# praveer13/zest

Measured on AMD Instinct MI355X. Metric: aggregate pull GB/s + P2P ratio, Llama-3.1-70B at 1/2/4/8 MI355X peers, higher is better.
Workload: dtype bf16

## Files before the change

csrc/gpu/compress.hip:

```cpp
#include <hip/hip_runtime.h>

#include <cstdint>
#include <cstdlib>

#include "zgpu.h"

namespace {

constexpr int kWave = 64;
constexpr int kWavesPerBlock = 4;
constexpr int kTabLog = 12;
constexpr uint32_t kTab = 1u << kTabLog;

__device__ __forceinline__ uint32_t lane_id() { return threadIdx.x & (kWave - 1); }

__device__ __forceinline__ uint32_t load_u32(const uint8_t* p) {
  const uintptr_t a = reinterpret_cast<uintptr_t>(p);
  const uint32_t k = uint32_t(a & 3);
  const uint32_t* w = reinterpret_cast<const uint32_t*>(a & ~uintptr_t(3));
  const uint32_t w0 = w[0];
  return k == 0 ? w0 : __builtin_amdgcn_alignbyte(w[1], w0, k);
}

__device__ __forceinline__ uint32_t put_len(uint8_t* o, uint32_t op, uint32_t r, uint32_t lane) {
  const uint32_t nff = r / 255;
  for (uint32_t i = lane; i < nff; i += kWave) o[op + i] = 0xFF;
  if (lane == 0) o[op + nff] = uint8_t(r - 255 * nff);
  return op + nff + 1;
}

__device__ __forceinline__ uint32_t emit(uint8_t* o, uint32_t op, const uint8_t* in, uint32_t lit0, uint32_t L,
                                         uint32_t off, uint32_t ml, uint32_t lane) {
  const uint32_t M = ml ? ml - 4 : 0;
  if (lane == 0) o[op] = uint8_t(((L < 15 ? L : 15) << 4) | (ml ? (M < 15 ? M : 15) : 0));
  ++op;
  if (L >= 15) op = put_len(o, op, L - 15, lane);
  for (uint32_t i = lane; i < L; i += kWave) o[op + i] = in[lit0 + i];
  op += L;
  if (ml) {
    if (lane == 0) {
      o[op] = uint8_t(off & 0xFF);
      o[op + 1] = uint8_t(off >> 8);
    }
    op += 2;
    if (M >= 15) op = put_len(o, op, M - 15, lane);
  }
  return op;
}

__global__ void __launch_bounds__(256) k_bg4_split(const uint8_t* __restrict__ data, const uint64_t* __restrict__ offs,
                                                   const uint32_t* __restrict__ lens, int n, uint8_t* __restrict__ out,
                                                   uint64_t slot) {
  const int c = __builtin_amdgcn_readfirstlane(int(blockIdx.x * kWavesPerBlock + (threadIdx.x >> 6)));
  if (c >= n) return;
  const uint32_t lane = lane_id(), len = lens[c];
  const uint8_t* s = data + offs[c];
  uint8_t* d = out + uint64_t(c) * slot;
  const uint32_t q = len >> 2, r = len & 3;
  const uint32_t g1 = q + (r > 0), g2 = g1 + q + (r > 1), g3 = g2 + q + (r > 2);
  for (uint32_t i = lane; i < len; i += kWave) {
    const uint32_t g = i & 3, j = i >> 2;
    const uint32_t base = g == 0 ? 0u : g == 1 ? g1 : g == 2 ? g2 : g3;
    d[base + j] = s[i];
  }
}

__global__ void __launch_bounds__(256) k_lz4_compress_v1(const uint8_t* __restrict__ data, const uint64_t* __restrict__ offs,
                                                      const uint32_t* __restrict__ lens, int n, uint64_t in_slot,
                                                      uint8_t* __restrict__ out, uint64_t out_slot,
                                                      uint32_t* __restrict__ out_len, uint32_t hc64, uint32_t hc256) {
  __shared__ unsigned long long tabs[kWavesPerBlock][kTab];
  const int wave = __builtin_amdgcn_readfirstlane(int(threadIdx.x >> 6));
  const int c = __builtin_amdgcn_readfirstlane(int(blockIdx.x * kWavesPerBlock + wave));
  if (c >= n) return;
  const uint32_t lane = lane_id();
  unsigned long long* tab = tabs[wave];
  for (uint32_t i = lane; i < kTab; i += kWave) tab[i] = 0;
  __builtin_amdgcn_wave_barrier();
  const uint32_t len = lens[c];
  const uint8_t* in = in_slot ? data + uint64_t(c) * in_slot : data + offs[c];
  uint8_t* o = out + uint64_t(c) * out_slot;
  uint32_t op = 11, ip = 0, anchor = 0;
  const uint32_t mend = len > 5 ? len - 5 : 0;
  while (ip + 12 <= len) {
    const uint32_t p = ip + lane;
    const bool ok = p + 12 <= len;
    const uint32_t v = ok ? load_u32(in + p) : 0;
    const uint32_t h = (v * 2654435761u) >> (32 - kTabLog);
    const unsigned long long e = ok ? tab[h] : 0ull;
    uint32_t cand = uint32_t(e >> 32) - 1;
    bool hit = ok && e != 0 && uint32_t(e) == v && cand < p && p - cand <= 65535u;
    uint32_t near = 0;
    for (int d = 32; d >= 1; --d) {
      const uint32_t u = __shfl_up(v, d, kWave);
      if (lane >= uint32_t(d) && u == v) near = d;
    }
    if (ok && near) {
      cand = p - near;
      hit = true;
    }
    const unsigned long long mask = __ballot(hit);
    const uint32_t passed = mask ? uint32_t(__builtin_ctzll(mask)) + 1 : uint32_t(kWave);
    __builtin_amdgcn_wave_barrier();
    if (ok && lane < passed) atomicMax(&tab[h], (static_cast<unsigned long long>(p + 1) << 32) | v);
    if (!mask) {
      ip += kWave;
      continue;
    }
    const int j = __builtin_ctzll(mask);
    uint32_t mp = ip + uint32_t(j);
    uint32_t mc = uint32_t(__builtin_amdgcn_readlane(int(cand), j));
    while (true) {
      const uint32_t room = (mp - anchor) < mc ? (mp - anchor) : mc;
      if (room == 0) break;
      const uint32_t k = lane + 1;
      const bool eq = k <= room && in[mp - k] == in[mc - k];
      const unsigned long long ne = __ballot(!eq);
      const uint32_t b = ne ? uint32_t(__builtin_ctzll(ne)) : uint32_t(kWave);
      mp -= b;
      mc -= b;
      if (b < uint32_t(kWave)) break;
    }
    const uint32_t maxlen = mend - mp;
    uint32_t ml = 4 + (ip + uint32_t(j) - mp);
    while (ml < maxlen) {
      const uint32_t k = ml + lane;
      const bool eq = k < maxlen && in[mc + k] == in[mp + k];
      const unsigned long long ne = __ballot(!eq);
      if (ne) {
        ml += uint32_t(__builtin_ctzll(ne));
        break;
      }
      ml += kWave;
    }
    if (ml > maxlen) ml = maxlen;
    op = emit(o, op, in, anchor, mp - anchor, mp - mc, ml, lane);
    ip = mp + ml;
    anchor = ip;
  }
  op = emit(o, op, in, anchor, len - anchor, 0, 0, lane);
  const uint32_t total = op + 4;
  if (total >= len) {
    if (lane == 0) out_len[c] = 0;
    return;
  }
  if (lane == 0) {
    const uint32_t bs = op - 11;
    const bool small = len <= 65536;
    const uint8_t hdr[11] = {0x04, 0x22, 0x4D, 0x18, 0x60, uint8_t(small ? 0x40 : 0x50),
                             uint8_t(small ? hc64 : hc256), uint8_t(bs), uint8_t(bs >> 8), uint8_t(bs >> 16),
                             uint8_t(bs >> 24)};
    for (int i = 0; i < 11; ++i) o[i] = hdr[i];
    for (int i = 0; i < 4; ++i) o[op + i] = 0;
    out_len[c] = total;
  }
}

constexpr uint32_t kTagBits = 14;
constexpr uint32_t kTagMask = (1u << kTagBits) - 1;
constexpr uint32_t kRing = 4096;
constexpr uint32_t kRingMask = kRing - 1;
constexpr uint32_t kFlush = 2048;
constexpr uint32_t kHdr = 11;

struct Staged {
  uint8_t* ring;
  uint8_t* g;
  uint32_t flushed;
};

__device__ __forceinline__ void ring_write(Staged& o, uint32_t end, uint32_t lane) {
  __builtin_amdgcn_wave_barrier();
  for (uint32_t pos = o.flushed + lane; pos < end; pos += kWave)
    if (pos >= kHdr) o.g[pos] = o.ring[pos & kRingMask];
  __builtin_amdgcn_wave_barrier();
}

__device__ __forceinline__ void maybe_flush(Staged& o, uint32_t op, uint32_t lane) {
  while (op - o.flushed >= kFlush) {
    ring_write(o, o.flushed + kFlush, lane);
    o.flushed += kFlush;
  }
}

__device__ __forceinline__ uint32_t put_len_s(Staged& o, uint32_t op, uint32_t r, uint32_t lane) {
  const uint32_t nff = r / 255;
  for (uint32_t i = lane; i < nff; i += kWave) o.ring[(op + i) & kRingMask] = 0xFF;
  if (lane == 0) o.ring[(op + nff) & kRingMask] = uint8_t(r - 255 * nff);
  return op + nff + 1;
}

__device__ __forceinline__ uint32_t emit_s(Staged& o, uint32_t op, const uint8_t* in, uint32_t lit0, uint32_t L,
                                           uint32_t off, uint32_t ml, uint32_t lane) {
  const uint32_t M = ml ? ml - 4 : 0;
  maybe_flush(o, op, lane);
  if (lane == 0) o.ring[op & kRingMask] = uint8_t(((L < 15 ? L : 15) << 4) | (ml ? (M < 15 ? M : 15) : 0));
  ++op;
  if (L >= 15) op = put_len_s(o, op, L - 15, lane);
  for (uint32_t b = 0; b < L; b += 1024) {
    maybe_flush(o, op + b, lane);
    const uint32_t n = L - b < 1024 ? L - b : 1024;
    for (uint32_t i = lane; i < n; i += kWave) o.ring[(op + b + i) & kRingMask] = in[lit0 + b + i];
  }
  op += L;
  if (ml) {
    maybe_flush(o, op, lane);
    if (lane == 0) {
      o.ring[op & kRingMask] = uint8_t(off & 0xFF);
      o.ring[(op + 1) & kRingMask] = uint8_t(off >> 8);
    }
    op += 2;
    if (M >= 15) op = put_len_s(o, op, M - 15, lane);
  }
  return op;
}

__global__ void __launch_bounds__(256) k_lz4_compress(const uint8_t* __restrict__ data, const uint64_t* __restrict__ offs,
                                                      const uint32_t* __restrict__ lens, int n, uint64_t in_slot,
                                                      uint8_t* __restrict__ out, uint64_t out_slot,
                                                      uint32_t* __restrict__ out_len, uint32_t hc64, uint32_t hc256) {
  __shared__ uint32_t tabs[kWavesPerBlock][kTab];
  __shared__ uint8_t rings[kWavesPerBlock][kRing];
  const int wave = __builtin_amdgcn_readfirstlane(int(threadIdx.x >> 6));
  const int c = __builtin_amdgcn_readfirstlane(int(blockIdx.x * kWavesPerBlock + wave));
  if (c >= n) return;
  const uint32_t lane = lane_id();
  uint32_t* tab = tabs[wave];
  for (uint32_t i = lane; i < kTab; i += kWave) tab[i] = 0;
  __builtin_amdgcn_wave_barrier();
  const uint32_t len = lens[c];
  const uint8_t* in = in_slot ? data + uint64_t(c) * in_slot : data + offs[c];
  Staged o{rings[wave], out + uint64_t(c) * out_slot, 0};
  uint32_t op = kHdr, ip = 0, anchor = 0;
  const uint32_t mend = len > 5 ? len - 5 : 0;
  while (ip + 12 <= len) {
    const uint32_t p = ip + lane;
    const bool ok = p + 12 <= len;
    const uint32_t v = ok ? load_u32(in + p) : 0;
    const uint32_t hv = v * 2654435761u;
    const uint32_t h = hv >> (32 - kTabLog);
    const uint32_t tag = hv & kTagMask;
    const uint32_t e = ok ? tab[h] : 0u;
    uint32_t cand = (e >> kTagBits) - 1;
    bool hit = ok && e != 0 && (e & kTagMask) == tag && cand < p && p - cand <= 65535u;
    if (hit) hit = load_u32(in + cand) == v;
    uint32_t near = 0;
    for (int d = 32; d >= 1; --d) {
      const uint32_t u = __shfl_up(v, d, kWave);
      if (lane >= uint32_t(d) && u == v) near = d;
    }
    if (ok && near) {
      cand = p - near;
      hit = true;
    }
    const unsigned long long mask = __ballot(hit);
    const uint32_t passed = mask ? uint32_t(__builtin_ctzll(mask)) + 1 : uint32_t(kWave);
    __builtin_amdgcn_wave_barrier();
    if (ok && lane < passed) atomicMax(&tab[h], ((p + 1) << kTagBits) | tag);
    if (!mask) {
      ip += kWave;
      continue;
    }
    const int j = __builtin_ctzll(mask);
    uint32_t mp = ip + uint32_t(j);
    uint32_t mc = uint32_t(__builtin_amdgcn_readlane(int(cand), j));
    while (true) {
      const uint32_t room = (mp - anchor) < mc ? (mp - anchor) : mc;
      if (room == 0) break;
      const uint32_t k = lane + 1;
      const bool eq = k <= room && in[mp - k] == in[mc - k];
      const unsigned long long ne = __ballot(!eq);
      const uint32_t b = ne ? uint32_t(__builtin_ctzll(ne)) : uint32_t(kWave);
      mp -= b;
      mc -= b;
      if (b < uint32_t(kWave)) break;
    }
    const uint32_t maxlen = mend - mp;
    uint32_t ml = 4 + (ip + uint32_t(j) - mp);
    while (ml < maxlen) {
      const uint32_t k = ml + lane;
      const bool eq = k < maxlen && in[mc + k] == in[mp + k];
      const unsigned long long ne = __ballot(!eq);
      if (ne) {
        ml += uint32_t(__builtin_ctzll(ne));
        break;
      }
      ml += kWave;
    }
    if (ml > maxlen) ml = maxlen;
    op = emit_s(o, op, in, anchor, mp - anchor, mp - mc, ml, lane);
    ip = mp + ml;
    anchor = ip;
  }
  op = emit_s(o, op, in, anchor, len - anchor, 0, 0, lane);
  const uint32_t total = op + 4;
  if (total >= len) {
    if (lane == 0) out_len[c] = 0;
    return;
  }
  maybe_flush(o, op, lane);
  if (lane < 4) o.ring[(op + lane) & kRingMask] = 0;
  ring_write(o, total, lane);
  if (lane == 0) {
    const uint32_t bs = op - kHdr;
    const bool small = len <= 65536;
    const uint8_t hdr[kHdr] = {0x04, 0x22, 0x4D, 0x18, 0x60, uint8_t(small ? 0x40 : 0x50),
                               uint8_t(small ? hc64 : hc256), uint8_t(bs), uint8_t(bs >> 8), uint8_t(bs >> 16),
                               uint8_t(bs >> 24)};
    for (uint32_t i = 0; i < kHdr; ++i) o.g[i] = hdr[i];
    out_len[c] = total;
  }
}

bool compress_v1() {
  const char* e = getenv("ZG_COMPRESS");
  return e && e[0] == 'v' && e[1] == '1';
}

__global__ void __launch_bounds__(256) k_pack_frames(const uint64_t* __restrict__ src, const uint32_t* __restrict__ clen,
                                                     const uint32_t* __restrict__ ulen, const uint8_t* __restrict__ scheme,
                                                     const uint64_t* __restrict__ out_off, int n, uint8_t* __restrict__ out) {
  const int c = __builtin_amdgcn_readfirstlane(int(blockIdx.x * kWavesPerBlock + (threadIdx.x >> 6)));
  if (c >= n) return;
  const uint32_t lane = lane_id(), cl = clen[c], ul = ulen[c];
  uint8_t* d = out + out_off[c];
  if (lane < 8) {
    const uint32_t b = lane == 0 ? 0u : lane < 4 ? (cl >> (8 * (lane - 1))) & 0xFF
                                  : lane == 4 ? scheme[c] : (ul >> (8 * (lane - 5))) & 0xFF;
    d[lane] = uint8_t(b);
  }
  const uint8_t* s = reinterpret_cast<const uint8_t*>(src[c]);
  for (uint32_t i = lane; i < cl; i += kWave) d[8 + i] = s[i];
}

}

extern "C" {

hipError_t zg_compress_chunks(const uint8_t* data, const uint64_t* offs, const uint32_t* lens, int n, int bg4,
                              uint8_t* scratch, uint64_t in_slot, uint8_t* out, uint64_t out_slot, uint32_t* out_len,
                              uint32_t hc64, uint32_t hc256, hipStream_t stream) {
  if (n <= 0) return hipSuccess;
  const dim3 grid((n + kWavesPerBlock - 1) / kWavesPerBlock);
  auto* kern = compress_v1() ? k_lz4_compress_v1 : k_lz4_compress;
  if (bg4) {
    hipLaunchKernelGGL(k_bg4_split, grid, dim3(256), 0, stream, data, offs, lens, n, scratch, in_slot);
    hipLaunchKernelGGL(kern, grid, dim3(256), 0, stream, scratch, offs, lens, n, in_slot, out, out_slot, out_len,
                       hc64, hc256);
  } else {
    hipLaunchKernelGGL(kern, grid, dim3(256), 0, stream, data, offs, lens, n, uint64_t(0), out, out_slot, out_len,
                       hc64, hc256);
  }
  return hipGetLastError();
}

hipError_t zg_pack_frames(const uint64_t* src, const uint32_t* clen, const uint32_t* ulen, const uint8_t* scheme,
                          const uint64_t* out_off, int n, uint8_t* out, hipStream_t stream) {
  if (n <= 0) return hipSuccess;
  hipLaunchKernelGGL(k_pack_frames, dim3((n + kWavesPerBlock - 1) / kWavesPerBlock), dim3(256), 0, stream, src, clen,
                     ulen, scheme, out_off, n, out);
  return hipGetLastError();
}

}
```

Baseline: 62.58.

## Stage LZ4 input through LDS ring and batch multiple matches per wave window

The GPU LZ4 compressor now streams each chunk's input through a shared-memory ring, prefetched one refill ahead, so hashing, candidate verification, match extension and literal copies mostly read LDS instead of global memory. The near-match shuffle scan is cut to 8 distances first and only widened when needed. Backward and forward extension use precomputed 4-byte windows before falling back to wave-wide byte loops. Short sequences are emitted in one lane-parallel store, and several matches can be handled per loaded window. Each block now runs one wave instead of four, which changes occupancy and adds more complex control flow with some risk of subtle encoding bugs.

```diff
diff --git a/csrc/gpu/compress.hip b/csrc/gpu/compress.hip
--- a/csrc/gpu/compress.hip
+++ b/csrc/gpu/compress.hip
@@ -190,17 +190,93 @@
   return op + nff + 1;
 }
 
-__device__ __forceinline__ uint32_t emit_s(Staged& o, uint32_t op, const uint8_t* in, uint32_t lit0, uint32_t L,
+#ifndef ZG_LZ4_INRING
+#define ZG_LZ4_INRING 1024
+#endif
+constexpr uint32_t kIn = ZG_LZ4_INRING;
+static_assert(kIn >= 1024 && (kIn & (kIn - 1)) == 0, "input ring: a power of two, at least two refills");
+constexpr uint32_t kInMask = kIn - 1;
+constexpr uint32_t kInDwMask = kIn / 4 - 1;
+constexpr uint32_t kRefill = 512;
+constexpr uint32_t kAhead = 128;
+
+struct Input {
+  const uint8_t* in;
+  const uint32_t* g32;
+  uint32_t* r32;
+  uint32_t k;
+  uint32_t ndw;
+  uint32_t lo, hi;
+  uint32_t pend0, pend1;
+};
+
+__device__ __forceinline__ void in_issue(Input& s, uint32_t lane) {
+  const uint32_t d = (s.hi >> 2) + lane;
+  s.pend0 = d < s.ndw ? s.g32[d] : 0u;
+  s.pend1 = d + kWave < s.ndw ? s.g32[d + kWave] : 0u;
+}
+
+__device__ __forceinline__ void in_commit(Input& s, uint32_t lane) {
+  const uint32_t d = (s.hi >> 2) + lane;
+  s.r32[d & kInDwMask] = s.pend0;
+  s.r32[(d + kWave) & kInDwMask] = s.pend1;
+  s.hi += kRefill;
+  if (s.hi - s.lo > kIn) s.lo = s.hi - kIn;
+  in_issue(s, lane);
+}
+
+__device__ __forceinline__ void in_ensure(Input& s, uint32_t a0, uint32_t lane) {
+  if (a0 > s.hi + kRefill) {
+    s.hi = (a0 - kWave) & ~3u;
+    s.lo = s.hi;
+    in_issue(s, lane);
+  }
+  while (s.hi < a0 + kAhead && s.hi < s.ndw * 4) in_commit(s, lane);
+  __builtin_amdgcn_wave_barrier();
+}
+
+__device__ __forceinline__ uint8_t in_byte(const Input& s, uint32_t p) {
+  const uint32_t a = p + s.k;
+  return (a >= s.lo && a < s.hi) ? reinterpret_cast<const uint8_t*>(s.r32)[a & kInMask] : s.in[p];
+}
+
+struct Cand {
+  uint32_t pre, val, f0, f1;
+};
+
+__device__ __forceinline__ Cand fetch_cand(const Input& s, uint32_t mc, bool want) {
+  const uint32_t a = mc + s.k, d = a >> 2, sh = a & 3;
+  uint32_t c[5];
+#pragma unroll
+  for (uint32_t i = 0; i < 5; ++i) c[i] = s.r32[(d - 1 + i) & kInDwMask];
+  const bool gone = want && (d ? d - 1 : 0u) * 4 < s.lo;
+  if (__ballot(gone)) {
+    if (gone) {
+#pragma unroll
+      for (uint32_t i = 0; i < 5; ++i) c[i] = d - 1 + i < s.ndw ? s.g32[d - 1 + i] : 0u;
+    }
+  }
+  return Cand{__builtin_amdgcn_alignbyte(c[1], c[0], sh), __builtin_amdgcn_alignbyte(c[2], c[1], sh),
+              __builtin_amdgcn_alignbyte(c[3], c[2], sh), __builtin_amdgcn_alignbyte(c[4], c[3], sh)};
+}
+
+__device__ __forceinline__ uint32_t emit_s(Staged& o, uint32_t op, const Input& in, uint32_t lit0, uint32_t L,
                                            uint32_t off, uint32_t ml, uint32_t lane) {
   const uint32_t M = ml ? ml - 4 : 0;
   maybe_flush(o, op, lane);
   if (lane == 0) o.ring[op & kRingMask] = uint8_t(((L < 15 ? L : 15) << 4) | (ml ? (M < 15 ? M : 15) : 0));
   ++op;
   if (L >= 15) op = put_len_s(o, op, L - 15, lane);
+  const uint8_t* r8 = reinterpret_cast<const uint8_t*>(in.r32);
   for (uint32_t b = 0; b < L; b += 1024) {
     maybe_flush(o, op + b, lane);
     const uint32_t n = L - b < 1024 ? L - b : 1024;
-    for (uint32_t i = lane; i < n; i += kWave) o.ring[(op + b + i) & kRingMask] = in[lit0 + b + i];
+    const uint32_t a = lit0 + b + in.k;
+    if (a >= in.lo && a + n <= in.hi) {
+      for (uint32_t i = lane; i < n; i += kWave) o.ring[(op + b + i) & kRingMask] = r8[(a + i) & kInMask];
+    } else {
+      for (uint32_t i = lane; i < n; i += kWave) o.ring[(op + b + i) & kRingMask] = in.in[lit0 + b + i];
+    }
   }
   op += L;
   if (ml) {
@@ -215,84 +291,159 @@
   return op;
 }
 
-__global__ void __launch_bounds__(256) k_lz4_compress(const uint8_t* __restrict__ data, const uint64_t* __restrict__ offs,
-                                                      const uint32_t* __restrict__ lens, int n, uint64_t in_slot,
-                                                      uint8_t* __restrict__ out, uint64_t out_slot,
-                                                      uint32_t* __restrict__ out_len, uint32_t hc64, uint32_t hc256) {
-  __shared__ uint32_t tabs[kWavesPerBlock][kTab];
-  __shared__ uint8_t rings[kWavesPerBlock][kRing];
-  const int wave = __builtin_amdgcn_readfirstlane(int(threadIdx.x >> 6));
-  const int c = __builtin_amdgcn_readfirstlane(int(blockIdx.x * kWavesPerBlock + wave));
+constexpr int kNearFirst = 8;
+
+__global__ void __launch_bounds__(kWave) k_lz4_compress(const uint8_t* __restrict__ data, const uint64_t* __restrict__ offs,
+                                                        const uint32_t* __restrict__ lens, int n, uint64_t in_slot,
+                                                        uint8_t* __restrict__ out, uint64_t out_slot,
+                                                        uint32_t* __restrict__ out_len, uint32_t hc64, uint32_t hc256) {
+  __shared__ uint32_t tab[kTab];
+  __shared__ uint8_t ring[kRing];
+  __shared__ uint32_t inring[kIn / 4];
+  const int c = int(blockIdx.x);
   if (c >= n) return;
-  const uint32_t lane = lane_id();
-  uint32_t* tab = tabs[wave];
+  const uint32_t lane = threadIdx.x;
   for (uint32_t i = lane; i < kTab; i += kWave) tab[i] = 0;
   __builtin_amdgcn_wave_barrier();
   const uint32_t len = lens[c];
   const uint8_t* in = in_slot ? data + uint64_t(c) * in_slot : data + offs[c];
-  Staged o{rings[wave], out + uint64_t(c) * out_slot, 0};
+  Input s;
+  s.in = in;
+  s.k = uint32_t(reinterpret_cast<uintptr_t>(in) & 3);
+  s.g32 = reinterpret_cast<const uint32_t*>(in - s.k);
+  s.r32 = inring;
+  s.ndw = len ? (s.k + len + 3) >> 2 : 0u;
+  s.lo = s.hi = 0;
+  in_issue(s, lane);
+  Staged o{ring, out + uint64_t(c) * out_slot, 0};
   uint32_t op = kHdr, ip = 0, anchor = 0;
   const uint32_t mend = len > 5 ? len - 5 : 0;
   while (ip + 12 <= len) {
-    const uint32_t p = ip + lane;
+    const uint32_t a0 = ip + s.k;
+    in_ensure(s, a0, lane);
+    const uint32_t p = ip + lane, a = a0 + lane, q = a >> 2, sh = a & 3;
     const bool ok = p + 12 <= len;
-    const uint32_t v = ok ? load_u32(in + p) : 0;
+    const uint32_t wm = s.r32[(q - 1) & kInDwMask], w0 = s.r32[q & kInDwMask], w1 = s.r32[(q + 1) & kInDwMask],
+                   w2 = s.r32[(q + 2) & kInDwMask], w3 = s.r32[(q + 3) & kInDwMask];
+    const uint32_t v = __builtin_amdgcn_alignbyte(w1, w0, sh);
     const uint32_t hv = v * 2654435761u;
     const uint32_t h = hv >> (32 - kTabLog);
     const uint32_t tag = hv & kTagMask;
-    const uint32_t e = ok ? tab[h] : 0u;
-    uint32_t cand = (e >> kTagBits) - 1;
-    bool hit = ok && e != 0 && (e & kTagMask) == tag && cand < p && p - cand <= 65535u;
-    if (hit) hit = load_u32(in + cand) == v;
-    uint32_t near = 0;
-    for (int d = 32; d >= 1; --d) {
+    const uint32_t vpre = __builtin_amdgcn_alignbyte(w0, wm, sh), vf0 = __builtin_amdgcn_alignbyte(w2, w1, sh),
+                   vf1 = __builtin_amdgcn_alignbyte(w3, w2, sh);
+    uint32_t near8 = 0;
+#pragma unroll
+    for (int d = kNearFirst; d >= 1; --d) {
       const uint32_t u = __shfl_up(v, d, kWave);
-      if (lane >= uint32_t(d) && u == v) near = d;
-    }
-    if (ok && near) {
-      cand = p - near;
-      hit = true;
-    }
-    const unsigned long long mask = __ballot(hit);
-    const uint32_t passed = mask ? uint32_t(__builtin_ctzll(mask)) + 1 : uint32_t(kWave);
-    __builtin_amdgcn_wave_barrier();
-    if (ok && lane < passed) atomicMax(&tab[h], ((p + 1) << kTagBits) | tag);
-    if (!mask) {
-      ip += kWave;
-      continue;
-    }
-    const int j = __builtin_ctzll(mask);
-    uint32_t mp = ip + uint32_t(j);
-    uint32_t mc = uint32_t(__builtin_amdgcn_readlane(int(cand), j));
+      if (lane >= uint32_t(d) && u == v) near8 = d;
+    }
+    uint32_t s0 = 0;
     while (true) {
+      const bool live = ok && lane >= s0;
+      const uint32_t e = live ? tab[h] : 0u;
+      uint32_t cand = (e >> kTagBits) - 1;
+      const bool tagged = live && e != 0 && (e & kTagMask) == tag && cand < p && p - cand <= 65535u;
+      const Cand cb = fetch_cand(s, cand, tagged);
+      const bool far = tagged && cb.val == v;
+      const unsigned long long mfar = __ballot(far);
+      const uint32_t jf = mfar ? uint32_t(__builtin_ctzll(mfar)) : uint32_t(kWave);
+      uint32_t near = near8 <= lane - s0 ? near8 : 0u;
+      if (jf - s0 > uint32_t(kNearFirst)) {
+        uint32_t nr = 0;
+        for (uint32_t d = jf - s0 < 32 ? jf - s0 : 32; d > uint32_t(kNearFirst); --d) {
+          const uint32_t u = __shfl_up(v, d, kWave);
+          if (lane >= s0 + d && u == v) nr = d;
+        }
+        if (!near) near = nr;
+      }
+      const unsigned long long mask = mfar | __ballot(live && near != 0);
+      if (!mask && s0) {
+        ip += s0;
+        break;
+      }
+      const uint32_t passed = mask ? uint32_t(__builtin_ctzll(mask)) + 1 : uint32_t(kWave);
+      __builtin_amdgcn_wave_barrier();
+      if (live && lane < passed) atomicMax(&tab[h], ((p + 1) << kTagBits) | tag);
+      if (!mask) {
+        ip += kWave;
+        break;
+      }
+      const int j = __builtin_ctzll(mask);
+      uint32_t mp = ip + uint32_t(j);
+      const uint32_t jnear = uint32_t(__builtin_amdgcn_readlane(int(near), j));
+      uint32_t mc;
+      Cand w;
+      if (jnear) {
+        mc = mp - jnear;
+        const Cand t = fetch_cand(s, mc, true);
+        w = Cand{uint32_t(__builtin_amdgcn_readfirstlane(int(t.pre))), 0u, uint32_t(__builtin_amdgcn_readfirstlane(int(t.f0))),
+                 uint32_t(__builtin_amdgcn_readfirstlane(int(t.f1)))};
+      } else {
+        mc = uint32_t(__builtin_amdgcn_readlane(int(cand), j));
+        w = Cand{uint32_t(__builtin_amdgcn_readlane(int(cb.pre), j)), 0u, uint32_t(__builtin_amdgcn_readlane(int(cb.f0), j)),
+                 uint32_t(__builtin_amdgcn_readlane(int(cb.f1), j))};
+      }
       const uint32_t room = (mp - anchor) < mc ? (mp - anchor) : mc;
-      if (room == 0) break;
-      const uint32_t k = lane + 1;
-      const bool eq = k <= room && in[mp - k] == in[mc - k];
-      const unsigned long long ne = __ballot(!eq);
-      const uint32_t b = ne ? uint32_t(__builtin_ctzll(ne)) : uint32_t(kWave);
-      mp -= b;
-      mc -= b;
-      if (b < uint32_t(kWave)) break;
-    }
-    const uint32_t maxlen = mend - mp;
-    uint32_t ml = 4 + (ip + uint32_t(j) - mp);
-    while (ml < maxlen) {
-      const uint32_t k = ml + lane;
-      const bool eq = k < maxlen && in[mc + k] == in[mp + k];
-      const unsigned long long ne = __ballot(!eq);
-      if (ne) {
-        ml += uint32_t(__builtin_ctzll(ne));
+      const uint32_t xb = uint32_t(__builtin_amdgcn_readlane(int(vpre), j)) ^ w.pre;
+      uint32_t nb = xb ? uint32_t(__builtin_clz(xb)) >> 3 : 4u;
+      const bool back_more = nb == 4 && room > 4;
+      if (nb > room) nb = room;
+      mp -= nb;
+      mc -= nb;
+      if (back_more) {
+        while (true) {
+          const uint32_t rm = (mp - anchor) < mc ? (mp - anchor) : mc;
+          if (rm == 0) break;
+          const uint32_t k = lane + 1;
+          const bool eq = k <= rm && in_byte(s, mp - k) == in_byte(s, mc - k);
+          const unsigned long long ne = __ballot(!eq);
+          const uint32_t b = ne ? uint32_t(__builtin_ctzll(ne)) : uint32_t(kWave);
+          mp -= b;
+          mc -= b;
+          if (b < uint32_t(kWave)) break;
+        }
+      }
+      const uint32_t maxlen = mend - mp;
+      uint32_t ml = 4 + (ip + uint32_t(j) - mp);
+      const uint32_t x0 = uint32_t(__builtin_amdgcn_readlane(int(vf0), j)) ^ w.f0;
+      const uint32_t x1 = uint32_t(__builtin_amdgcn_readlane(int(vf1), j)) ^ w.f1;
+      if (x0) {
+        ml += uint32_t(__builtin_ctz(x0)) >> 3;
+      } else if (x1) {
+        ml += 4 + (uint32_t(__builtin_ctz(x1)) >> 3);
+      } else {
+        ml += 8;
+        while (ml < maxlen) {
+          const uint32_t k = ml + lane;
+          const bool eq = k < maxlen && in_byte(s, mc + k) == in_byte(s, mp + k);
+          const unsigned long long ne = __ballot(!eq);
+          if (ne) {
+            ml += uint32_t(__builtin_ctzll(ne));
+            break;
+          }
+          ml += kWave;
+        }
+      }
+      if (ml > maxlen) ml = maxlen;
+      const uint32_t L = mp - anchor, off = mp - mc;
+      if (anchor >= ip && L < 15 && ml < 19) {
+        maybe_flush(o, op, lane);
+        const uint32_t r = (lane - (anchor - ip)) & (kWave - 1);
+        const uint32_t b = r < L ? v : r == L ? ((L << 4) | (ml - 4)) : r == L + 1 ? off : off >> 8;
+        if (r < L + 3) o.ring[(r < L ? op + 1 + r : r == L ? op : op + r) & kRingMask] = uint8_t(b);
+        op += L + 3;
+      } else {
+        op = emit_s(o, op, s, anchor, L, off, ml, lane);
+      }
+      anchor = mp + ml;
+      s0 = anchor - ip;
+      if (s0 > kWave - 20 || anchor + 12 > len) {
+        ip = anchor;
         break;
       }
-      ml += kWave;
-    }
-    if (ml > maxlen) ml = maxlen;
-    op = emit_s(o, op, in, anchor, mp - anchor, mp - mc, ml, lane);
-    ip = mp + ml;
-    anchor = ip;
-  }
-  op = emit_s(o, op, in, anchor, len - anchor, 0, 0, lane);
+    }
+  }
+  op = emit_s(o, op, s, anchor, len - anchor, 0, 0, lane);
   const uint32_t total = op + 4;
   if (total >= len) {
     if (lane == 0) out_len[c] = 0;
@@ -342,15 +493,13 @@
                               uint32_t hc64, uint32_t hc256, hipStream_t stream) {
   if (n <= 0) return hipSuccess;
   const dim3 grid((n + kWavesPerBlock - 1) / kWavesPerBlock);
-  auto* kern = compress_v1() ? k_lz4_compress_v1 : k_lz4_compress;
-  if (bg4) {
-    hipLaunchKernelGGL(k_bg4_split, grid, dim3(256), 0, stream, data, offs, lens, n, scratch, in_slot);
-    hipLaunchKernelGGL(kern, grid, dim3(256), 0, stream, scratch, offs, lens, n, in_slot, out, out_slot, out_len,
-                       hc64, hc256);
-  } else {
-    hipLaunchKernelGGL(kern, grid, dim3(256), 0, stream, data, offs, lens, n, uint64_t(0), out, out_slot, out_len,
-                       hc64, hc256);
-  }
+  const bool v1 = compress_v1();
+  auto* kern = v1 ? k_lz4_compress_v1 : k_lz4_compress;
+  const dim3 kgrid = v1 ? grid : dim3(n), kblock = v1 ? dim3(256) : dim3(kWave);
+  const uint8_t* src = bg4 ? scratch : data;
+  if (bg4) hipLaunchKernelGGL(k_bg4_split, grid, dim3(256), 0, stream, data, offs, lens, n, scratch, in_slot);
+  hipLaunchKernelGGL(kern, kgrid, kblock, 0, stream, src, offs, lens, n, bg4 ? in_slot : uint64_t(0), out, out_slot,
+                     out_len, hc64, hc256);
   return hipGetLastError();
 }
 
```

Result: no change. 62.51 (-0.1%).
